# UltronAI/Depth-VO-Feat

Hardware: AMD Instinct MI355X
Metric: KITTI 256x832 stereo-seq samples/sec fwd+bwd (higher is better)
Workload: dtype f32

## Files before the change

### depth-vo-feat_amd/csrc/conv.hip

```cpp
#include "dvf_common.h"
#include "conv_op.h"
#include "conv_pipe_host.h"
#include "conv_gather.h"
#include "conv_wgrad.h"
#include "wgrad_pipe.h"

namespace {

__device__ __forceinline__ float act_grad(float g, float yv, int act, float alpha, float beta) {
    if (act == DVF_ACT_RELU) return (yv > 0.f) ? g : 0.f;
    if (act == DVF_ACT_SIGMOID_AFFINE) {
        const float sg = (yv - beta) / alpha;
        return g * alpha * sg * (1.f - sg);
    }
    return g;
}

template <bool VEC>
__global__ __launch_bounds__(256) void act_bwd_kernel(const float *__restrict__ dy, const float *__restrict__ y,
                                                      float *__restrict__ dpre, float *dbias, int C, int HW, int act,
                                                      float alpha, float beta, int chunks, float *part = nullptr, int nper = 0) {
    __shared__ float red[4];
    const int plane = blockIdx.x / chunks, chunk = blockIdx.x - plane * chunks;
    const int c = plane % C;
// ... 263 lines not shown
    const int rc = plan_gather(op, pl);
    return rc ? rc : pl.ws_floats;
}

struct DgradSeg {
    int s, off;
    ConvOp op;
    bool packed;
    PipePlan plan;
    int64_t packed_off;
};

template <class F>
int for_each_dgrad_seg(const dvf_conv_desc *d, const int *seg_channels, int nseg, bool use_pipe, F visit) {
    DgradSeg v;
    v.off = 0; v.packed_off = 0;
    for (v.s = 0; v.s < nseg; ++v.s) {
        int rc = make_dgrad_op(d, v.off, seg_channels[v.s], v.op);
        v.packed = false;
        if (use_pipe) {
            if (rc) return rc;
            rc = plan_pipe(v.op, v.plan);
            if (rc && rc != DVF_ERR_UNSUPPORTED) return rc;
            v.packed = !rc;
        }
        rc = visit(v);
        if (rc) return rc;
        if (v.packed) v.packed_off += v.plan.packed_floats;
        v.off += seg_channels[v.s];
    }
// ... 13 lines not shown
        if (rc) return rc;
        rc = plan_pipe(op, pl);
        if (rc == DVF_ERR_UNSUPPORTED && want_ws) return unpacked_ws_floats(op, fwd_direct(d, nseg) != FWD_NONE);
        return rc ? rc : (want_ws ? pl.ws_floats : pl.packed_floats);
    }
    if (op_kind != 1) return DVF_ERR_INVALID_ARG;
    int64_t total = 0, wmax = 0;
    int nsup = 0;
    rc = for_each_dgrad_seg(d, seg_channels, nseg, true, [&](const DgradSeg &v) -> int {
        int64_t wf = 0;
        if (v.packed) {
            total += v.plan.packed_floats;
            wf = v.plan.ws_floats;
            ++nsup;
        } else if (want_ws) {
            wf = unpacked_ws_floats(v.op, dvf_head_seg_dgrad_applicable(d, v.op.M));
            if (wf < 0) return (int)wf;
        }
        wmax = wf > wmax ? wf : wmax;
        return DVF_OK;
    });
    if (rc) return rc;
    if (!nsup && !want_ws) return DVF_ERR_UNSUPPORTED;
    return want_ws ? wmax : total;
}

WgradArgs wgrad_args(const dvf_conv_desc *d, const float *const *in_segs, const int *seg_channels, int s, const float *dpre,
                     float *dw) {
    int off = 0;
    for (int i = 0; i < s; ++i) off += seg_channels[i];
    const int segc = s < 0 ? d->C_in : seg_channels[s];
// ... 307 lines not shown
    }
    return fwd_unpacked(d, op, io, seg_channels, nseg, w, ws, ws_floats, st);
}

int dvf_conv2d_dgrad(const dvf_conv_desc *d, const float *dpre, const float *packed, const float *w, float *const *din_segs,
                     const int *seg_channels, int nseg, float *ws, int64_t ws_floats, const float *const *mask_segs,
                     void *stream) {
    dvf_plan_reset();
    int rc = check_desc(d);
    if (rc) return rc;
    rc = check_segs(d, seg_channels, nseg);
    if (rc) return rc;
    if (!dpre || !w || !din_segs) return DVF_ERR_INVALID_ARG;
    hipStream_t st = dvf_stream(stream);
    auto mask = [&](int s) -> const float * { return mask_segs ? mask_segs[s] : nullptr; };
    if (dvf_head_dgrad_applicable(d, nseg) || (dvf_head_applicable(d, nseg) && !packed))
        return din_segs[0] ? dvf_head_dgrad(d, dpre, w, din_segs[0], st, mask(0)) : DVF_OK;
    return for_each_dgrad_seg(d, seg_channels, nseg, packed != nullptr, [&](const DgradSeg &v) -> int {
        if (!din_segs[v.s]) return DVF_OK;
        const ConvIO io{&dpre, nullptr, din_segs[v.s], mask(v.s)};
        int r = v.packed ? run_pipe(v.op, v.plan, io, packed + v.packed_off, ws, ws_floats, st) : DVF_ERR_UNSUPPORTED;
        if (r == DVF_ERR_UNSUPPORTED) r = dgrad_unpacked(d, v.op, io, w, ws, ws_floats, st);
        return r;
    });
}

int dvf_conv2d_pack_jobs(const dvf_conv_desc *d, const int *seg_channels, int nseg, int op_kind, const float *w, float *packed,
                         void *jobs_host, int max_jobs, int *blocks_out, int *lds_bytes_out) {
    static_assert(sizeof(PackArgs) <= DVF_PACK_JOB_BYTES, "DVF_PACK_JOB_BYTES too small");
    int rc = check_desc(d);
    if (rc) return rc;
// ... 54 lines not shown
```

### depth-vo-feat_amd/csrc/conv_head.h

```cpp
#pragma once
#include "dvf_common.h"
bool dvf_head_applicable(const dvf_conv_desc *d, int nseg);
bool dvf_head_fwd_applicable(const dvf_conv_desc *d, int nseg);
bool dvf_head_dgrad_applicable(const dvf_conv_desc *d, int nseg);
int dvf_head_fwd(const dvf_conv_desc *d, const float *in, const float *w, const float *bias, float *out, hipStream_t st);
bool dvf_head_wide_applicable(const dvf_conv_desc *d, int nseg);
int dvf_head_fwd_segs(const dvf_conv_desc *d, const float *const *in_segs, const int *seg_channels, int nseg, const float *w,
                      const float *bias, float *out, hipStream_t st);
int dvf_head_dgrad(const dvf_conv_desc *d, const float *dpre, const float *w, float *din, hipStream_t st, const float *mask = nullptr);
int dvf_head_wgrad(const dvf_conv_desc *d, const float *in, const float *dpre, float *dw, int accumulate, hipStream_t st,
                   float *ws = nullptr, int64_t ws_floats = 0);
int64_t dvf_head_wgrad_ws_floats(const dvf_conv_desc *d);
bool dvf_head_seg_dgrad_applicable(const dvf_conv_desc *d, int segc);
int dvf_head_seg_dgrad(const dvf_conv_desc *d, const float *dpre, const float *w, float *din, int seg_off, int segc,
                       hipStream_t st, const float *mask = nullptr);
bool dvf_dconvt_applicable(const dvf_conv_desc *d, int nseg);
int dvf_dconvt_fwd(const dvf_conv_desc *d, const float *in, const float *w, const float *bias, float *out, hipStream_t st);
```

### depth-vo-feat_amd/csrc/conv_head.hip

```cpp
#include "conv_head.h"
#include "conv_epilogue.h"

namespace {

using dvfp::apply_act;

constexpr int HT_W = 64, HT_H = 4;
constexpr int HP_W = HT_W + 2, HP_H = HT_H + 2;
constexpr int HCK = 8;

__device__ __forceinline__ void stage_tile(float *lds, const float *__restrict__ src, int64_t plane, int nch, int H, int W,
                                           int y0, int x0) {
    for (int e = threadIdx.x; e < nch * HP_H * HP_W; e += 256) {
        const int ch = e / (HP_H * HP_W), r = e - ch * (HP_H * HP_W), py = r / HP_W, px = r - py * HP_W;
        const int y = y0 + py - 1, x = x0 + px - 1;
        lds[e] = (y >= 0 && y < H && x >= 0 && x < W) ? src[ch * plane + (int64_t)y * W + x] : 0.f;
    }
}

template <int ROWS, int MO, class WK>
__device__ __forceinline__ void taps9(const float (&v)[ROWS + 2][3], WK wk, float (&acc)[ROWS][MO]) {
#pragma unroll
    for (int m = 0; m < MO; ++m)
#pragma unroll
        for (int k = 0; k < 9; ++k) {
            const float w = wk(m, k);
#pragma unroll
            for (int r = 0; r < ROWS; ++r) acc[r][m] = fmaf(w, v[k / 3 + r][k % 3], acc[r][m]);
        }
}

constexpr int FT_H = 8;
constexpr int HEAD_MAX_SEGS = 3;
struct HeadSegs {
    const float *p[HEAD_MAX_SEGS];
    int c[HEAD_MAX_SEGS];
    int n;
};
template <int MO, int HCKT, int FTH>
__global__ __launch_bounds__(256) void head_fwd_kernel(const HeadSegs in, const float *__restrict__ w,
                                                       const float *__restrict__ bias, float *__restrict__ out, int C, int H,
                                                       int W, int tilesX, int act, float alpha, float beta, int ws_m, int ws_c,
                                                       int flip, const float *__restrict__ mask) {
    constexpr int ROWS = FTH / 4, FPH = FTH + 2, FPN = FPH * HP_W, FLD = (FPN + 255) / 256;
    extern __shared__ __attribute__((aligned(16))) float wsh[];
    float *tile = wsh + ((MO * C * 9 + 3) & ~3);
    for (int e = threadIdx.x; e < MO * C * 9; e += 256) {
        const int m = e / (C * 9), r = e - m * (C * 9), c = r / 9, k = r - c * 9;
        const float wv = w[(int64_t)m * ws_m + (int64_t)c * ws_c + (flip ? 8 - k : k)];
        if (MO == 16) wsh[(c * MO + m) * 9 + k] = wv;
        else wsh[e] = wv;
    }
    const int n = blockIdx.y, tY = blockIdx.x / tilesX, tX = blockIdx.x - tY * tilesX;
    const int y0 = tY * FTH, x0 = tX * HT_W;
    const int lx = threadIdx.x & (HT_W - 1), ly = (threadIdx.x >> 6) * ROWS;
    const int64_t plane = (int64_t)H * W;
    int soff[FLD];
#pragma unroll
    for (int i = 0; i < FLD; ++i) {
        const int e = threadIdx.x + 256 * i, py = e / HP_W, px = e - py * HP_W;
        const int y = y0 + py - 1, x = x0 + px - 1;
        soff[i] = (e < FPN && y >= 0 && y < H && x >= 0 && x < W) ? y * W + x : -1;
    }
    float acc[ROWS][MO];
#pragma unroll
    for (int m = 0; m < MO; ++m)
// ... 22 lines not shown
        for (int ch = 0; ch < HCKT; ++ch)
#pragma unroll
            for (int i = 0; i < FLD; ++i) {
                const int e = threadIdx.x + 256 * i;
                if (e < FPN) tile[ch * FPN + e] = stg[ch][i];
            }
        __syncthreads();
        if (sg2 < in.n) issue(sg2, cs2);
        auto hood = [&](int ch, float (&v)[ROWS + 2][3]) __attribute__((always_inline)) {
            const float *t = tile + ch * FPN + ly * HP_W + lx;
#pragma unroll
            for (int a = 0; a < ROWS + 2; ++a)
#pragma unroll
                for (int b = 0; b < 3; ++b) v[a][b] = t[a * HP_W + b];
        };
        if constexpr (MO != 16) {
            auto wlds = [&](int c) __attribute__((always_inline)) {
                return [=](int m, int k) __attribute__((always_inline)) { return wsh[(m * C + c) * 9 + k]; };
            };
            float part[3][ROWS][MO];
#pragma unroll
            for (int q = 0; q < 3; ++q)
#pragma unroll
                for (int r = 0; r < ROWS; ++r)
#pragma unroll
                    for (int m = 0; m < MO; ++m) part[q][r][m] = 0.f;
            int ch = 0;
            for (; ch + 4 <= nch; ch += 4) {
                float v4[4][ROWS + 2][3];
#pragma unroll
                for (int q = 0; q < 4; ++q) hood(ch + q, v4[q]);
#pragma unroll
                for (int q = 0; q < 4; ++q)
#pragma unroll
                    for (int m = 0; m < MO; ++m) {
                        const float *wm = wsh + (m * C + cg + ch + q) * 9;
#pragma unroll
                        for (int k = 0; k < 9; ++k) {
                            const float wk = wm[k];
#pragma unroll
                            for (int r = 0; r < ROWS; ++r) {
                                if (q == 0) acc[r][m] = fmaf(wk, v4[q][k / 3 + r][k % 3], acc[r][m]);
                                else part[q - 1][r][m] = fmaf(wk, v4[q][k / 3 + r][k % 3], part[q - 1][r][m]);
                            }
                        }
                    }
            }
            for (; ch < nch; ++ch) {
                float v[ROWS + 2][3];
                hood(ch, v);
                taps9<ROWS, MO>(v, wlds(cg + ch), acc);
            }
#pragma unroll
            for (int r = 0; r < ROWS; ++r)
#pragma unroll
                for (int m = 0; m < MO; ++m) acc[r][m] += (part[0][r][m] + part[1][r][m]) + part[2][r][m];
        } else {
            for (int ch = 0; ch < nch; ++ch) {
                float v[ROWS + 2][3];
                hood(ch, v);
                typedef float f4h __attribute__((ext_vector_type(4)));
                const f4h *wq = reinterpret_cast<const f4h *>(wsh + (cg + ch) * (MO * 9));
                f4h wr[MO * 9 / 4];
#pragma unroll
                for (int q = 0; q < MO * 9 / 4; ++q) wr[q] = wq[q];
                taps9<ROWS, MO>(v, [&](int m, int k) __attribute__((always_inline)) { return wr[(m * 9 + k) >> 2][(m * 9 + k) & 3]; }, acc);
            }
        }
        cg += nch; sg = sg2; cs = cs2;
    }
    const int x = x0 + lx;
#pragma unroll
    for (int r = 0; r < ROWS; ++r) {
        const int y = y0 + ly + r;
        if (y < H && x < W) {
            if (mask) {
#pragma unroll
                for (int m = 0; m < MO; ++m) {
                    const int64_t idx = ((int64_t)n * MO + m) * plane + (int64_t)y * W + x;
                    out[idx] = mask[idx] > 0.f ? acc[r][m] : 0.f;
                }
            } else {
#pragma unroll
                for (int m = 0; m < MO; ++m)
                    out[((int64_t)n * MO + m) * plane + (int64_t)y * W + x] = apply_act(acc[r][m], act, alpha, beta);
            }
        }
    }
}

template <int MO>
__global__ __launch_bounds__(256) void head_dgrad_kernel(const float *__restrict__ dpre, const float *__restrict__ w,
                                                         float *__restrict__ din, int C, int H, int W, int tilesX,
                                                         const float *__restrict__ mask) {
    __shared__ float tile[MO * HP_H * HP_W];
    extern __shared__ __attribute__((aligned(16))) float wsh[];
    constexpr int WPC = (MO * 9 + 3) & ~3;
    for (int e = threadIdx.x; e < C * MO * 9; e += 256) {
        const int c = e / (MO * 9), r = e - c * (MO * 9), m = r / 9, k = r - m * 9;
        wsh[c * WPC + r] = w[((int64_t)m * C + c) * 9 + k];
    }
    const int n = blockIdx.y, tY = blockIdx.x / tilesX, tX = blockIdx.x - tY * tilesX;
    const int y0 = tY * HT_H, x0 = tX * HT_W;
    const int lx = threadIdx.x & (HT_W - 1), ly = threadIdx.x >> 6;
    const int64_t plane = (int64_t)H * W;
    stage_tile(tile, dpre + (int64_t)n * MO * plane, plane, MO, H, W, y0, x0);
    __syncthreads();
    float g[MO][9];
#pragma unroll
    for (int m = 0; m < MO; ++m)
#pragma unroll
        for (int a = 0; a < 3; ++a)
#pragma unroll
            for (int b = 0; b < 3; ++b) g[m][a * 3 + b] = tile[m * (HP_H * HP_W) + (ly + 2 - a) * HP_W + (lx + 2 - b)];
    const int y = y0 + ly, x = x0 + lx;
    if (y >= H || x >= W) return;
    const int64_t base = (int64_t)n * C * plane + (int64_t)y * W + x;
    float *dst = din + base;
    const float *mk = mask ? mask + base : nullptr;
    for (int c0 = 0; c0 < C; c0 += 4) {
        float sv[4], mv[4];
#pragma unroll
        for (int q = 0; q < 4; ++q) {
            const int c = min(c0 + q, C - 1);
            mv[q] = mk ? mk[c * plane] : 1.f;
            const float *wc = wsh + c * WPC;
            float s = 0.f;
#pragma unroll
            for (int m = 0; m < MO; ++m)
#pragma unroll
                for (int k = 0; k < 9; ++k) s = fmaf(wc[m * 9 + k], g[m][k], s);
            sv[q] = s;
        }
#pragma unroll
        for (int q = 0; q < 4; ++q)
            if (c0 + q < C) dst[(c0 + q) * plane] = (mv[q] > 0.f) ? sv[q] : 0.f;
    }
}

template <bool VEC>
__device__ __forceinline__ void hw_load4(const float *__restrict__ p, int x0, int W, bool ok, float (&v)[4]) {
    if (VEC) {
        typedef float f4 __attribute__((ext_vector_type(4)));
        f4 t = {0.f, 0.f, 0.f, 0.f};
        if (ok) t = *reinterpret_cast<const f4 *>(p);
#pragma unroll
        for (int j = 0; j < 4; ++j) v[j] = t[j];
    } else {
#pragma unroll
        for (int j = 0; j < 4; ++j) v[j] = (ok && x0 + j < W) ? p[j] : 0.f;
    }
// ... 95 lines not shown
            const int64_t o = ((int64_t)m * C + c0 + c) * 9 + t;
            if (part) part[(int64_t)blockIdx.y * MO * C * 9 + o] = s;
            else atomicAdd(&dw[o], s);
        }
    }
}

__global__ __launch_bounds__(256) void head_wgrad_finish_kernel(const float *__restrict__ part, float *dw, int n, int groups) {
    const int e = blockIdx.x * 256 + threadIdx.x;
    if (e >= n) return;
    float s = 0.f;
    for (int g = 0; g < groups; ++g) s += part[(int64_t)g * n + e];
    dw[e] += s;
}


template <int CO, int K>
__global__ __launch_bounds__(256) void dconvt_s2_fwd_kernel(const float *__restrict__ in, const float *__restrict__ w,
                                                            const float *__restrict__ bias, float *__restrict__ out, int C, int H,
                                                            int W, int OH, int OW, int act, float alpha, float beta) {
    extern __shared__ __attribute__((aligned(16))) float wlds[];
    constexpr int WPC = CO * K * K;
    static_assert(WPC % 4 == 0, "weights of one input channel are read in 16-byte pieces");
    typedef float f4w __attribute__((ext_vector_type(4)));
    for (int e = threadIdx.x; e < C * WPC / 4; e += 256)
        reinterpret_cast<f4w *>(wlds)[e] = reinterpret_cast<const f4w *>(w)[e];
    __syncthreads();
    const int x = blockIdx.x * 64 + (threadIdx.x & 63), y = blockIdx.y * 4 + (threadIdx.x >> 6), n = blockIdx.z;
    const bool inside = x < W && y < H;
    const bool rok[3] = {y - 1 >= 0 && y - 1 < H, y < H, y + 1 < H}, cok[3] = {x - 1 >= 0 && x - 1 < W, x < W, x + 1 < W};
// ... 51 lines not shown
            } else {
                if (X < OW) q[0] = r0;
                if (X + 1 < OW) q[1] = r1;
            }
        }
    }
}

}

bool dvf_head_applicable(const dvf_conv_desc *d, int nseg) {
    return nseg == 1 && !d->transposed && d->KH == 3 && d->KW == 3 && d->stride == 1 && d->pad == 1 && d->C_out >= 1 &&
           d->C_out <= 4 && d->H_out == d->H_in && d->W_out == d->W_in && d->C_in >= 4 && d->C_in * d->C_out <= 1024 &&
           dvf_tune("DVF_NO_HEAD") == nullptr;
}
bool dvf_head_fwd_applicable(const dvf_conv_desc *d, int nseg) {
    static const int maxc = dvf_tune("DVF_HEAD_FWD_MAXC") ? atoi(dvf_tune("DVF_HEAD_FWD_MAXC")) : 127;
    return dvf_head_applicable(d, nseg) && d->C_in <= maxc;
}
bool dvf_head_dgrad_applicable(const dvf_conv_desc *d, int nseg) {
    static const int maxc = dvf_tune("DVF_HEAD_DGRAD_MAXC") ? atoi(dvf_tune("DVF_HEAD_DGRAD_MAXC")) : 32;
    return dvf_head_applicable(d, nseg) && d->C_in <= maxc;
}

bool dvf_dconvt_applicable(const dvf_conv_desc *d, int nseg) {
    const bool k3 = d->KH == 3 && d->KW == 3, k4 = d->KH == 4 && d->KW == 4;
    return nseg == 1 && d->transposed && d->stride == 2 && d->pad == 1 && (k3 || k4) && d->C_out == 16 &&
           d->C_in >= 8 && d->C_in <= 64 && d->H_out <= 2 * d->H_in && d->W_out <= 2 * d->W_in &&
           (int64_t)d->H_in * d->W_in >= 64 * 64 && (int64_t)d->N * d->C_out * d->H_out * d->W_out < ((int64_t)1 << 31) &&
           dvf_tune("DVF_NO_DCONVT") == nullptr;
}

int dvf_dconvt_fwd(const dvf_conv_desc *d, const float *in, const float *w, const float *bias, float *out, hipStream_t st) {
    const dim3 grid(cdiv(d->W_in, 64), cdiv(d->H_in, 4), d->N);
    const size_t lds = (size_t)d->C_in * d->C_out * d->KH * d->KW * 4;
    if ((reinterpret_cast<uintptr_t>(w) & 15) != 0 || lds > 64 * 1024) return DVF_ERR_UNSUPPORTED;
#define DCONVT(CO, K) dconvt_s2_fwd_kernel<CO, K><<<grid, 256, lds, st>>>(in, w, bias, out, d->C_in, d->H_in, d->W_in, d->H_out, d->W_out, d->act, d->alpha, d->beta)
    if (d->KH == 3) DCONVT(16, 3);
    else DCONVT(16, 4);
#undef DCONVT
    DVF_LAUNCH_CHECK();
    dvf_plan_note(DVF_K_DCONVT_FWD, d->C_out, d->KH);
    return DVF_OK;
}

#define HEAD_CASE(N, ...) case N: { constexpr int MO = N; __VA_ARGS__; } break;
#define HEAD_DISPATCH(MOV, CALL, ...)             \
    switch (MOV) {                               \
        HEAD_CASE(1, CALL) HEAD_CASE(2, CALL) HEAD_CASE(3, CALL) HEAD_CASE(4, CALL) __VA_ARGS__ \
        default: return DVF_ERR_UNSUPPORTED;     \
    }

static int head_fwd_launch(int MOv, const HeadSegs &in, const float *w, const float *bias, float *out, int C, int N, int H, int W,
                           int act, float alpha, float beta, int ws_m, int ws_c, int flip, const float *mask, hipStream_t st) {
    const bool lowres = (int64_t)N * H * W <= (int64_t)4 * 64 * 208 && MOv <= 4 && C >= 32;
    const int FTH = lowres ? 4 : FT_H, HCKT = lowres ? 32 : HCK;
    const int tilesX = cdiv(W, HT_W), tilesY = cdiv(H, FTH);
    const dim3 grid(tilesX * tilesY, N);
    const size_t lds = ((size_t)((MOv * C * 9 + 3) & ~3) + (size_t)HCKT * (FTH + 2) * HP_W) * 4;
#define HEAD_FWD_GO(HC, FH) head_fwd_kernel<MO, HC, FH><<<grid, 256, lds, st>>>(in, w, bias, out, C, H, W, tilesX, act, alpha, beta, ws_m, ws_c, flip, mask)
    if (lowres) {
        static bool big[5] = {false, false, false, false, false};
        HEAD_DISPATCH(MOv, {
            if (lds > 64 * 1024 && !big[MO]) {
                if (hipFuncSetAttribute(reinterpret_cast<const void *>(&head_fwd_kernel<MO, 32, 4>), hipFuncAttributeMaxDynamicSharedMemorySize, 160 * 1024) != hipSuccess) return DVF_ERR_LAUNCH;
                big[MO] = true;
            }
            HEAD_FWD_GO(32, 4); });
    } else {
        HEAD_DISPATCH(MOv, (HEAD_FWD_GO(8, 8)), HEAD_CASE(16, (HEAD_FWD_GO(8, 8))));
    }
#undef HEAD_FWD_GO
    DVF_LAUNCH_CHECK();
    return DVF_OK;
}

int dvf_head_fwd(const dvf_conv_desc *d, const float *in, const float *w, const float *bias, float *out, hipStream_t st) {
    const int one = d->C_in;
    return dvf_head_fwd_segs(d, &in, &one, 1, w, bias, out, st);
}

bool dvf_head_wide_applicable(const dvf_conv_desc *d, int nseg) {
    return nseg >= 1 && nseg <= HEAD_MAX_SEGS && !d->transposed && d->KH == 3 && d->KW == 3 && d->stride == 1 && d->pad == 1 &&
           d->C_out == 16 && d->C_in <= 24 && d->H_out == d->H_in && d->W_out == d->W_in &&
           (int64_t)d->H_in * d->W_in >= 64 * 64 && dvf_tune("DVF_NO_HEAD") == nullptr && dvf_tune("DVF_NO_WIDE_HEAD") == nullptr;
}

// ... 19 lines not shown

int dvf_head_seg_dgrad(const dvf_conv_desc *d, const float *dpre, const float *w, float *din, int seg_off, int segc,
                       hipStream_t st, const float *mask) {
    const float *wseg = w + (int64_t)seg_off * 9;
    HeadSegs in{};
    for (int s = 0; s < HEAD_MAX_SEGS; ++s) { in.p[s] = dpre; in.c[s] = s == 0 ? d->C_out : 0; }
    in.n = 1;
    const int rc = head_fwd_launch(segc, in, wseg, nullptr, din, d->C_out, d->N, d->H_in, d->W_in, DVF_ACT_NONE, 1.f, 0.f, 9,
                                   d->C_in * 9, 1, mask, st);
    if (rc) return rc;
    dvf_plan_note(DVF_K_HEAD_SEG_DGRAD, segc);
    return DVF_OK;
}

int dvf_head_dgrad(const dvf_conv_desc *d, const float *dpre, const float *w, float *din, hipStream_t st, const float *mask) {
    const int tilesX = cdiv(d->W_in, HT_W), tilesY = cdiv(d->H_in, HT_H);
    const dim3 grid(tilesX * tilesY, d->N);
    HEAD_DISPATCH(d->C_out, (head_dgrad_kernel<MO><<<grid, 256, (size_t)d->C_in * ((MO * 9 + 3) & ~3) * 4, st>>>(
                                dpre, w, din, d->C_in, d->H_in, d->W_in, tilesX, mask)));
    DVF_LAUNCH_CHECK();
    dvf_plan_note(DVF_K_HEAD_DGRAD, d->C_out);
    return DVF_OK;
}

struct HeadWgradGrid { int cch, RS, xgroups, segs, chunks, groups; int64_t units; };
static HeadWgradGrid head_wgrad_grid(const dvf_conv_desc *d) {
    HeadWgradGrid g;
    g.xgroups = cdiv(d->W_in, 4);
    auto blocks = [&](int cch, int rs) {
        return (int64_t)cdiv(d->C_in, cch) * (((int64_t)d->N * cdiv(d->H_in, rs) * g.xgroups + 255) / 256);
    };
    const int min_blocks = 400, max_blocks = 1024;
    g.cch = (d->C_out <= 2 && blocks(4, 8) >= 512) ? 4 : 2;
    g.RS = 8;
// ... 41 lines not shown
```

### depth-vo-feat_amd/csrc/conv_op.h

```cpp
#pragma once
#include "dvf_common.h"
#include "conv_head.h"

namespace {

inline int ilog2(int v) { int l = 0; while ((1 << l) < v) ++l; return l; }
inline int roundup(int v, int q) { return (v + q - 1) / q * q; }

struct ClassSpec { int OS, py, px, IS, by, bx, TA, TB, OHc, OWc; int tapmap[49]; };

struct ConvOp {
    int nseg, segC[DVF_MAX_SEGS];
    int w_mode;
    int Mtot, Rtot, KK, m_base, M;
    int N, IH, IW, OH, OW;
    int act;
    float alpha, beta;
    ClassSpec cls[4];
    int ncls;
    bool covers;
    int Tmax, TAmax, TBmax, OHc, OWc;
    bool head_fwd;
};

struct ConvIO {
    const float *const *in;
    const float *bias;
    float *out;
    const float *mask;
};

int check_desc(const dvf_conv_desc *d) {
    if (!d) return DVF_ERR_INVALID_ARG;
    if (d->N <= 0 || d->C_in <= 0 || d->C_out <= 0 || d->H_in <= 0 || d->W_in <= 0 || d->H_out <= 0 || d->W_out <= 0)
        return DVF_ERR_INVALID_ARG;
    if (d->KH < 1 || d->KW < 1 || d->KH > 7 || d->KW > 7 || (d->stride != 1 && d->stride != 2) || d->pad < 0)
        return DVF_ERR_INVALID_ARG;
// ... 55 lines not shown
    for (int i = 0; i < op.ncls; ++i) {
        const ClassSpec &c = op.cls[i];
        op.Tmax = max(op.Tmax, c.TA * c.TB); op.TAmax = max(op.TAmax, c.TA); op.TBmax = max(op.TBmax, c.TB);
        op.OHc = max(op.OHc, c.OHc); op.OWc = max(op.OWc, c.OWc);
    }
    return op.ncls >= 1 ? DVF_OK : DVF_ERR_UNSUPPORTED;
}

int make_fwd_op(const dvf_conv_desc *d, const int *seg_channels, int nseg, ConvOp &op) {
    op = ConvOp{};
    for (int s = 0; s < nseg; ++s) op.segC[s] = seg_channels[s];
    op.nseg = nseg; op.M = d->C_out;
    op.N = d->N; op.IH = d->H_in; op.IW = d->W_in; op.OH = d->H_out; op.OW = d->W_out;
    op.act = d->act; op.alpha = d->alpha; op.beta = d->beta;
    op.KK = d->KH * d->KW; op.m_base = 0; op.Mtot = d->C_out; op.Rtot = d->C_in;
    op.head_fwd = !dvf_head_fwd_applicable(d, nseg) && dvf_head_applicable(d, nseg);
    op.w_mode = d->transposed ? 1 : 0;
    return set_classes(d, !d->transposed, op);
}

int make_dgrad_op(const dvf_conv_desc *d, int off, int segc, ConvOp &op) {
    op = ConvOp{};
    op.segC[0] = d->C_out; op.nseg = 1; op.M = segc;
    op.N = d->N; op.IH = d->H_out; op.IW = d->W_out; op.OH = d->H_in; op.OW = d->W_in;
    op.act = DVF_ACT_NONE;
    op.KK = d->KH * d->KW; op.m_base = off; op.Mtot = d->C_in; op.Rtot = d->C_out;
    op.head_fwd = false;
    op.w_mode = d->transposed ? 0 : 1;
    return set_classes(d, d->transposed != 0, op);
}

}
```

### depth-vo-feat_amd/csrc/conv_pipe_host.h

```cpp
#pragma once
#include <string.h>
#include "dvf_common.h"
#include "conv_pipe.h"
#include "conv_op.h"

namespace {

using dvfp::PClass;
using dvfp::PipeArgs;
using dvfp::PipeGeo;
using dvfp::pipe_geo;
using dvfp::PIPE_MAXNPI;
using dvfp::OUT_FUSED;
using dvfp::OUT_ATOMIC;
using dvfp::OUT_WS;

struct alignas(8) PackArgsBody {
    const float *w;
    float *wp;
    int w_mode;
    int Mtot, Rtot, KK, m_base, M;
    int nseg, segC[DVF_MAX_SEGS];
    int ncls, NCH, CK, MB, VW, TBU;
    int TB[4], TA[4];
// ... 271 lines not shown
                    const double cov = (double)cdiv(OWc, BW) * BW * cdiv(OHc, BH) * BH * cdiv(N, BN) * BN;
                    const double narrow = (SW >= 16 ? 0.0 : (SW == 8 ? 0.12 : 0.3)) + (BW >= 32 ? 0.0 : 0.08);
                    const double cost = cov * (1.0 + narrow + 0.02 * lsh + 0.02 * lsn) + 1e-3 * (BW + BH);
                    if (cost < best.cov) best = PipeTiles{lsw, lsh, TGX, TGY, TGN, BN, cost};
                }
            }
        }
    }
    return best;
}


int plan_pipe(const ConvOp &op, PipePlan &pl) {
    if (op.ncls < 1) return DVF_ERR_UNSUPPORTED;
    const ClassSpec *cls = op.cls;
    const int ncls = op.ncls, Tmax = op.Tmax, TAmax = op.TAmax, TBmax = op.TBmax, OHc = op.OHc, OWc = op.OWc;
    const bool head_fwd = op.head_fwd;
    PipeArgs &a = pl.a;
    a = PipeArgs{};
    for (int s = 0; s < op.nseg; ++s) a.segC[s] = op.segC[s];
    a.nseg = op.nseg; a.M = op.M;
    a.N = op.N; a.IH = op.IH; a.IW = op.IW; a.OH = op.OH; a.OW = op.OW;
    a.act = op.act; a.alpha = op.alpha; a.beta = op.beta;
    a.ncls = ncls; a.OS = cls[0].OS; a.IS = cls[0].IS;
    const PipeOverride ov = pipe_override();
    static const int smallm = dvf_tune("DVF_PIPE_SMALLM") ? atoi(dvf_tune("DVF_PIPE_SMALLM")) : 0;
    int ctot = 0;
    for (int s = 0; s < a.nseg; ++s) ctot += a.segC[s];
    static const int headc = dvf_tune("DVF_PIPE_HEADC") ? atoi(dvf_tune("DVF_PIPE_HEADC")) : 128;
    const bool wide_head = head_fwd && a.M <= 4 && ncls == 1 && ctot >= headc && Tmax == 9;
    const bool small_ok = a.M > 16 || wide_head || (!(smallm & 8) && a.M <= 16 && ncls > 1) ||
                          ((smallm & 2) && a.M <= 16) || ((smallm & 4) && a.M > 16);
    if (a.M <= 32 && !ov.on && !small_ok) return DVF_ERR_UNSUPPORTED;
    if (ov.on && ov.KS < 0) return DVF_ERR_UNSUPPORTED;
    int maxc = 0;
    for (int s = 0; s < a.nseg; ++s) maxc = a.segC[s] > maxc ? a.segC[s] : maxc;
    const int64_t px = (int64_t)OHc * OWc;
    int TBU = TBmax;
    if (TBU == 6) TBU = 7;
    if (TBU > 7) return DVF_ERR_UNSUPPORTED;
    int MT = a.M > 32 ? 2 : 1;
    int BN = 1;
    if (px <= 64) { while (BN < a.N && BN * px < 128 && BN < 32) BN *= 2; }
    int WM = 1;
    if (px * BN <= 64 && a.M >= 128) WM = 2;
    int NT = 2;
// ... 195 lines not shown
```

Measured before the change: 646.3.

## Replace LDS-tiled head conv kernels with register-streaming fwd/dgrad kernels

Adds new streaming kernels for the 1-4 output-channel head convolutions, covering both forward and dgrad. Each lane computes a 4-wide by RS-row output strip held in registers, with double-buffered channel loads and weights broadcast via readlane. Forward can split channels across waves with an LDS reduction, and dgrad splits channels across grid.y, so small spatial sizes still fill the GPU. Every head layer, including wide ones, now routes to these kernels instead of the packed pipe GEMM or the LDS-tile kernels. This risks slower paths for large-C layers that previously used the pipe, and adds more register pressure.

New measurement: 651.0, median of 6. No clear change (+0.7%).

```diff
diff --git a/depth-vo-feat_amd/csrc/conv.hip b/depth-vo-feat_amd/csrc/conv.hip
--- a/depth-vo-feat_amd/csrc/conv.hip
+++ b/depth-vo-feat_amd/csrc/conv.hip
@@ -301,6 +301,7 @@
 template <class F>
 int for_each_dgrad_seg(const dvf_conv_desc *d, const int *seg_channels, int nseg, bool use_pipe, F visit) {
     DgradSeg v;
+    use_pipe = use_pipe && !dvf_head_applicable(d, nseg);
     v.off = 0; v.packed_off = 0;
     for (v.s = 0; v.s < nseg; ++v.s) {
         int rc = make_dgrad_op(d, v.off, seg_channels[v.s], v.op);
@@ -344,7 +345,7 @@
             wf = v.plan.ws_floats;
             ++nsup;
         } else if (want_ws) {
-            wf = unpacked_ws_floats(v.op, dvf_head_seg_dgrad_applicable(d, v.op.M));
+            wf = unpacked_ws_floats(v.op, dvf_head_applicable(d, nseg) || dvf_head_seg_dgrad_applicable(d, v.op.M));
             if (wf < 0) return (int)wf;
         }
         wmax = wf > wmax ? wf : wmax;
@@ -682,7 +683,7 @@
     if (!dpre || !w || !din_segs) return DVF_ERR_INVALID_ARG;
     hipStream_t st = dvf_stream(stream);
     auto mask = [&](int s) -> const float * { return mask_segs ? mask_segs[s] : nullptr; };
-    if (dvf_head_dgrad_applicable(d, nseg) || (dvf_head_applicable(d, nseg) && !packed))
+    if (dvf_head_applicable(d, nseg))
         return din_segs[0] ? dvf_head_dgrad(d, dpre, w, din_segs[0], st, mask(0)) : DVF_OK;
     return for_each_dgrad_seg(d, seg_channels, nseg, packed != nullptr, [&](const DgradSeg &v) -> int {
         if (!din_segs[v.s]) return DVF_OK;
diff --git a/depth-vo-feat_amd/csrc/conv_head.h b/depth-vo-feat_amd/csrc/conv_head.h
--- a/depth-vo-feat_amd/csrc/conv_head.h
+++ b/depth-vo-feat_amd/csrc/conv_head.h
@@ -1,8 +1,6 @@
 #pragma once
 #include "dvf_common.h"
 bool dvf_head_applicable(const dvf_conv_desc *d, int nseg);
-bool dvf_head_fwd_applicable(const dvf_conv_desc *d, int nseg);
-bool dvf_head_dgrad_applicable(const dvf_conv_desc *d, int nseg);
 int dvf_head_fwd(const dvf_conv_desc *d, const float *in, const float *w, const float *bias, float *out, hipStream_t st);
 bool dvf_head_wide_applicable(const dvf_conv_desc *d, int nseg);
 int dvf_head_fwd_segs(const dvf_conv_desc *d, const float *const *in_segs, const int *seg_channels, int nseg, const float *w,
diff --git a/depth-vo-feat_amd/csrc/conv_head.hip b/depth-vo-feat_amd/csrc/conv_head.hip
--- a/depth-vo-feat_amd/csrc/conv_head.hip
+++ b/depth-vo-feat_amd/csrc/conv_head.hip
@@ -5,18 +5,9 @@
 
 using dvfp::apply_act;
 
-constexpr int HT_W = 64, HT_H = 4;
-constexpr int HP_W = HT_W + 2, HP_H = HT_H + 2;
+constexpr int HT_W = 64;
+constexpr int HP_W = HT_W + 2;
 constexpr int HCK = 8;
-
-__device__ __forceinline__ void stage_tile(float *lds, const float *__restrict__ src, int64_t plane, int nch, int H, int W,
-                                           int y0, int x0) {
-    for (int e = threadIdx.x; e < nch * HP_H * HP_W; e += 256) {
-        const int ch = e / (HP_H * HP_W), r = e - ch * (HP_H * HP_W), py = r / HP_W, px = r - py * HP_W;
-        const int y = y0 + py - 1, x = x0 + px - 1;
-        lds[e] = (y >= 0 && y < H && x >= 0 && x < W) ? src[ch * plane + (int64_t)y * W + x] : 0.f;
-    }
-}
 
 template <int ROWS, int MO, class WK>
 __device__ __forceinline__ void taps9(const float (&v)[ROWS + 2][3], WK wk, float (&acc)[ROWS][MO]) {
@@ -45,11 +36,10 @@
     constexpr int ROWS = FTH / 4, FPH = FTH + 2, FPN = FPH * HP_W, FLD = (FPN + 255) / 256;
     extern __shared__ __attribute__((aligned(16))) float wsh[];
     float *tile = wsh + ((MO * C * 9 + 3) & ~3);
+    static_assert(MO == 16, "the 1-4 channel layers run head_stream_fwd_kernel");
     for (int e = threadIdx.x; e < MO * C * 9; e += 256) {
         const int m = e / (C * 9), r = e - m * (C * 9), c = r / 9, k = r - c * 9;
-        const float wv = w[(int64_t)m * ws_m + (int64_t)c * ws_c + (flip ? 8 - k : k)];
-        if (MO == 16) wsh[(c * MO + m) * 9 + k] = wv;
-        else wsh[e] = wv;
+        wsh[(c * MO + m) * 9 + k] = w[(int64_t)m * ws_m + (int64_t)c * ws_c + (flip ? 8 - k : k)];
     }
     const int n = blockIdx.y, tY = blockIdx.x / tilesX, tX = blockIdx.x - tY * tilesX;
     const int y0 = tY * FTH, x0 = tX * HT_W;
@@ -102,58 +92,15 @@
 #pragma unroll
                 for (int b = 0; b < 3; ++b) v[a][b] = t[a * HP_W + b];
         };
-        if constexpr (MO != 16) {
-            auto wlds = [&](int c) __attribute__((always_inline)) {
-                return [=](int m, int k) __attribute__((always_inline)) { return wsh[(m * C + c) * 9 + k]; };
-            };
-            float part[3][ROWS][MO];
-#pragma unroll
-            for (int q = 0; q < 3; ++q)
-#pragma unroll
-                for (int r = 0; r < ROWS; ++r)
-#pragma unroll
-                    for (int m = 0; m < MO; ++m) part[q][r][m] = 0.f;
-            int ch = 0;
-            for (; ch + 4 <= nch; ch += 4) {
-                float v4[4][ROWS + 2][3];
-#pragma unroll
-                for (int q = 0; q < 4; ++q) hood(ch + q, v4[q]);
-#pragma unroll
-                for (int q = 0; q < 4; ++q)
-#pragma unroll
-                    for (int m = 0; m < MO; ++m) {
-                        const float *wm = wsh + (m * C + cg + ch + q) * 9;
-#pragma unroll
-                        for (int k = 0; k < 9; ++k) {
-                            const float wk = wm[k];
-#pragma unroll
-                            for (int r = 0; r < ROWS; ++r) {
-                                if (q == 0) acc[r][m] = fmaf(wk, v4[q][k / 3 + r][k % 3], acc[r][m]);
-                                else part[q - 1][r][m] = fmaf(wk, v4[q][k / 3 + r][k % 3], part[q - 1][r][m]);
-                            }
-                        }
-                    }
-            }
-            for (; ch < nch; ++ch) {
-                float v[ROWS + 2][3];
-                hood(ch, v);
-                taps9<ROWS, MO>(v, wlds(cg + ch), acc);
-            }
-#pragma unroll
-            for (int r = 0; r < ROWS; ++r)
-#pragma unroll
-                for (int m = 0; m < MO; ++m) acc[r][m] += (part[0][r][m] + part[1][r][m]) + part[2][r][m];
-        } else {
-            for (int ch = 0; ch < nch; ++ch) {
-                float v[ROWS + 2][3];
-                hood(ch, v);
-                typedef float f4h __attribute__((ext_vector_type(4)));
-                const f4h *wq = reinterpret_cast<const f4h *>(wsh + (cg + ch) * (MO * 9));
-                f4h wr[MO * 9 / 4];
-#pragma unroll
-                for (int q = 0; q < MO * 9 / 4; ++q) wr[q] = wq[q];
-                taps9<ROWS, MO>(v, [&](int m, int k) __attribute__((always_inline)) { return wr[(m * 9 + k) >> 2][(m * 9 + k) & 3]; }, acc);
-            }
+        for (int ch = 0; ch < nch; ++ch) {
+            float v[ROWS + 2][3];
+            hood(ch, v);
+            typedef float f4h __attribute__((ext_vector_type(4)));
+            const f4h *wq = reinterpret_cast<const f4h *>(wsh + (cg + ch) * (MO * 9));
+            f4h wr[MO * 9 / 4];
+#pragma unroll
+            for (int q = 0; q < MO * 9 / 4; ++q) wr[q] = wq[q];
+            taps9<ROWS, MO>(v, [&](int m, int k) __attribute__((always_inline)) { return wr[(m * 9 + k) >> 2][(m * 9 + k) & 3]; }, acc);
         }
         cg += nch; sg = sg2; cs = cs2;
     }
@@ -174,55 +121,6 @@
                     out[((int64_t)n * MO + m) * plane + (int64_t)y * W + x] = apply_act(acc[r][m], act, alpha, beta);
             }
         }
-    }
-}
-
-template <int MO>
-__global__ __launch_bounds__(256) void head_dgrad_kernel(const float *__restrict__ dpre, const float *__restrict__ w,
-                                                         float *__restrict__ din, int C, int H, int W, int tilesX,
-                                                         const float *__restrict__ mask) {
-    __shared__ float tile[MO * HP_H * HP_W];
-    extern __shared__ __attribute__((aligned(16))) float wsh[];
-    constexpr int WPC = (MO * 9 + 3) & ~3;
-    for (int e = threadIdx.x; e < C * MO * 9; e += 256) {
-        const int c = e / (MO * 9), r = e - c * (MO * 9), m = r / 9, k = r - m * 9;
-        wsh[c * WPC + r] = w[((int64_t)m * C + c) * 9 + k];
-    }
-    const int n = blockIdx.y, tY = blockIdx.x / tilesX, tX = blockIdx.x - tY * tilesX;
-    const int y0 = tY * HT_H, x0 = tX * HT_W;
-    const int lx = threadIdx.x & (HT_W - 1), ly = threadIdx.x >> 6;
-    const int64_t plane = (int64_t)H * W;
-    stage_tile(tile, dpre + (int64_t)n * MO * plane, plane, MO, H, W, y0, x0);
-    __syncthreads();
-    float g[MO][9];
-#pragma unroll
-    for (int m = 0; m < MO; ++m)
-#pragma unroll
-        for (int a = 0; a < 3; ++a)
-#pragma unroll
-            for (int b = 0; b < 3; ++b) g[m][a * 3 + b] = tile[m * (HP_H * HP_W) + (ly + 2 - a) * HP_W + (lx + 2 - b)];
-    const int y = y0 + ly, x = x0 + lx;
-    if (y >= H || x >= W) return;
-    const int64_t base = (int64_t)n * C * plane + (int64_t)y * W + x;
-    float *dst = din + base;
-    const float *mk = mask ? mask + base : nullptr;
-    for (int c0 = 0; c0 < C; c0 += 4) {
-        float sv[4], mv[4];
-#pragma unroll
-        for (int q = 0; q < 4; ++q) {
-            const int c = min(c0 + q, C - 1);
-            mv[q] = mk ? mk[c * plane] : 1.f;
-            const float *wc = wsh + c * WPC;
-            float s = 0.f;
-#pragma unroll
-            for (int m = 0; m < MO; ++m)
-#pragma unroll
-                for (int k = 0; k < 9; ++k) s = fmaf(wc[m * 9 + k], g[m][k], s);
-            sv[q] = s;
-        }
-#pragma unroll
-        for (int q = 0; q < 4; ++q)
-            if (c0 + q < C) dst[(c0 + q) * plane] = (mv[q] > 0.f) ? sv[q] : 0.f;
     }
 }
 
@@ -348,6 +246,251 @@
     dw[e] += s;
 }
 
+
+__device__ __forceinline__ int64_t hs_block() { return (int64_t)(blockIdx.x & 7) * (gridDim.x >> 3) + (blockIdx.x >> 3); }
+
+constexpr int hs_cb(int MO, int RS) { return RS >= 4 ? (MO <= 2 ? 2 : 1) : RS == 2 ? 2 : 4; }
+
+template <bool VEC>
+__device__ __forceinline__ void hs_row6(const float *__restrict__ p, const float *__restrict__ safe, int x0, int W, bool ok,
+                                        float (&x)[6]) {
+    const bool l = ok && x0 > 0, r = ok && x0 + 4 < W;
+    const float vl = *(l ? p - 1 : safe), vr = *(r ? p + 4 : safe);
+    if (VEC) {
+        typedef float f4 __attribute__((ext_vector_type(4)));
+        const f4 t = *reinterpret_cast<const f4 *>(ok ? p : safe);
+#pragma unroll
+        for (int j = 0; j < 4; ++j) x[1 + j] = ok ? t[j] : 0.f;
+    } else {
+#pragma unroll
+        for (int j = 0; j < 4; ++j) {
+            const bool okj = ok && x0 + j < W;
+            const float t = *(okj ? p + j : safe);
+            x[1 + j] = okj ? t : 0.f;
+        }
+    }
+    x[0] = l ? vl : 0.f;
+    x[5] = r ? vr : 0.f;
+}
+
+template <int MO, int RS, bool VEC>
+__global__ __launch_bounds__(256) void head_stream_fwd_kernel(const float *__restrict__ in, const float *__restrict__ w,
+                                                              const float *__restrict__ bias, float *__restrict__ out, int C,
+                                                              int H, int W, int xgroups, int segs, int64_t units, int KS, int act,
+                                                              float alpha, float beta, int ws_m, int ws_c, int flip,
+                                                              const float *__restrict__ mask) {
+    constexpr int CB = hs_cb(MO, RS), NR = RS + 2, NA = RS * 4 * MO;
+    typedef float f4 __attribute__((ext_vector_type(4)));
+    extern __shared__ __attribute__((aligned(16))) float red[];
+    const int wave = __builtin_amdgcn_readfirstlane(threadIdx.x >> 6), lane = threadIdx.x & 63;
+    const int ks = wave & (KS - 1), ug = wave / KS;
+    if (hs_block() * (256 / KS) >= units) return;
+    const int64_t u = (hs_block() * (4 / KS) + ug) * 64 + lane;
+    const bool live = u < units;
+    const int upi = segs * xgroups;
+    const int n = live ? (int)(u / upi) : 0, q = live ? (int)(u - (int64_t)n * upi) : 0;
+    const int seg = q / xgroups, xg = q - seg * xgroups;
+    const int y0 = seg * RS, x0 = xg * 4;
+    const int64_t plane = (int64_t)H * W;
+    const int cper = (C + KS - 1) / KS, cb = ks * cper, ce = min(C, cb + cper);
+    const int64_t ibase = (int64_t)n * C * plane + x0;
+    bool yok[NR];
+#pragma unroll
+    for (int i = 0; i < NR; ++i) yok[i] = live && y0 - 1 + i >= 0 && y0 - 1 + i < H;
+    auto load = [&](int c0, float (&x)[CB][NR][6]) __attribute__((always_inline)) {
+#pragma unroll
+        for (int b = 0; b < CB; ++b) {
+            const bool okc = c0 + b < ce;
+#pragma unroll
+            for (int i = 0; i < NR; ++i)
+                hs_row6<VEC>(in + ibase + (int64_t)(c0 + b) * plane + (int64_t)(y0 - 1 + i) * W, in, x0, W, okc && yok[i], x[b][i]);
+        }
+    };
+    const int wl = min(lane, MO * 9 - 1), wm = wl / 9;
+    const int64_t woff = (int64_t)wm * ws_m + (flip ? 8 - (wl - wm * 9) : wl - wm * 9);
+    auto load_w = [&](int c0, float (&wv)[CB]) __attribute__((always_inline)) {
+#pragma unroll
+        for (int b = 0; b < CB; ++b) wv[b] = w[(int64_t)min(c0 + b, ce - 1) * ws_c + woff];
+    };
+    float acc[RS][4][MO];
+#pragma unroll
+    for (int m = 0; m < MO; ++m) {
+        const float b0 = (bias && ks == 0) ? bias[m] : 0.f;
+#pragma unroll
+        for (int r = 0; r < RS; ++r)
+#pragma unroll
+            for (int j = 0; j < 4; ++j) acc[r][j][m] = b0;
+    }
+    auto fma = [&](int c0, const float (&x)[CB][NR][6], const float (&wv)[CB]) __attribute__((always_inline)) {
+#pragma unroll
+        for (int b = 0; b < CB; ++b) {
+            if (c0 + b >= ce) continue;
+            float wk[MO][9];
+#pragma unroll
+            for (int m = 0; m < MO; ++m)
+#pragma unroll
+                for (int k = 0; k < 9; ++k) wk[m][k] = __int_as_float(__builtin_amdgcn_readlane(__float_as_int(wv[b]), m * 9 + k));
+#pragma unroll
+            for (int m = 0; m < MO; ++m)
+#pragma unroll
+                for (int ta = 0; ta < 3; ++ta)
+#pragma unroll
+                    for (int tb = 0; tb < 3; ++tb)
+#pragma unroll
+                        for (int r = 0; r < RS; ++r)
+#pragma unroll
+                            for (int j = 0; j < 4; ++j)
+                                acc[r][j][m] = fmaf(wk[m][ta * 3 + tb], x[b][r + ta][j + tb], acc[r][j][m]);
+        }
+    };
+    float xa[CB][NR][6], xb[CB][NR][6], wa[CB], wb[CB];
+    load_w(cb, wa);
+    load(cb, xa);
+    for (int c0 = cb; c0 < ce; c0 += 2 * CB) {
+        load_w(c0 + CB, wb);
+        load(c0 + CB, xb);
+        fma(c0, xa, wa);
+        load_w(c0 + 2 * CB, wa);
+        load(c0 + 2 * CB, xa);
+        fma(c0 + CB, xb, wb);
+    }
+    if (KS > 1) {
+        if (ks > 0) {
+            float *r = red + (int64_t)(ug * (KS - 1) + ks - 1) * NA * 64 + lane;
+#pragma unroll
+            for (int a = 0; a < NA; ++a) r[a * 64] = acc[a / (4 * MO)][(a / MO) & 3][a % MO];
+        }
+        __syncthreads();
+        if (ks > 0) return;
+        for (int k = 1; k < KS; ++k) {
+            const float *r = red + (int64_t)(ug * (KS - 1) + k - 1) * NA * 64 + lane;
+#pragma unroll
+            for (int a = 0; a < NA; ++a) acc[a / (4 * MO)][(a / MO) & 3][a % MO] += r[a * 64];
+        }
+    }
+    if (!live) return;
+#pragma unroll
+    for (int r = 0; r < RS; ++r) {
+        const int y = y0 + r;
+        if (y >= H) continue;
+#pragma unroll
+        for (int m = 0; m < MO; ++m) {
+            const int64_t idx = ((int64_t)n * MO + m) * plane + (int64_t)y * W + x0;
+            float o[4];
+            if (mask) {
+                float mv[4];
+                hw_load4<VEC>(mask + idx, x0, W, true, mv);
+#pragma unroll
+                for (int j = 0; j < 4; ++j) o[j] = mv[j] > 0.f ? acc[r][j][m] : 0.f;
+            } else {
+#pragma unroll
+                for (int j = 0; j < 4; ++j) o[j] = apply_act(acc[r][j][m], act, alpha, beta);
+            }
+            if (VEC) {
+                f4 t = {o[0], o[1], o[2], o[3]};
+                *reinterpret_cast<f4 *>(out + idx) = t;
+            } else {
+#pragma unroll
+                for (int j = 0; j < 4; ++j)
+                    if (x0 + j < W) out[idx + j] = o[j];
+            }
+        }
+    }
+}
+
+template <int MO, bool VEC>
+__global__ __launch_bounds__(256) void head_stream_dgrad_kernel(const float *__restrict__ dpre, const float *__restrict__ w,
+                                                                float *__restrict__ din, int C, int H, int W, int xgroups,
+                                                                int64_t units, int cper, const float *__restrict__ mask) {
+    constexpr int CQ = 4;
+    typedef float f4 __attribute__((ext_vector_type(4)));
+    if (hs_block() * 256 >= units) return;
+    const int64_t u = hs_block() * 256 + threadIdx.x;
+    const bool live = u < units;
+    const int upi = H * xgroups;
+    const int n = live ? (int)(u / upi) : 0, q = live ? (int)(u - (int64_t)n * upi) : 0;
+    const int y = q / xgroups, xg = q - y * xgroups, x0 = xg * 4;
+    const int64_t plane = (int64_t)H * W;
+    float g[MO][3][6];
+#pragma unroll
+    for (int m = 0; m < MO; ++m)
+#pragma unroll
+        for (int a = 0; a < 3; ++a) {
+            const int r = y - 1 + a;
+            hs_row6<VEC>(dpre + ((int64_t)n * MO + m) * plane + (int64_t)r * W + x0, dpre, x0, W, live && r >= 0 && r < H, g[m][a]);
+        }
+    const int cb = blockIdx.y * cper, ce = min(C, cb + cper);
+    const int64_t base = (int64_t)n * C * plane + (int64_t)y * W + x0;
+    auto load_mask = [&](int c0, float (&mv)[CQ][4]) __attribute__((always_inline)) {
+#pragma unroll
+        for (int b = 0; b < CQ; ++b) {
+            const bool ok = mask && live && c0 + b < ce;
+            const float *p = mask + base + (int64_t)(c0 + b) * plane;
+            if (VEC) {
+                const f4 t = *reinterpret_cast<const f4 *>(ok ? p : dpre);
+#pragma unroll
+                for (int j = 0; j < 4; ++j) mv[b][j] = ok ? t[j] : 1.f;
+            } else {
+#pragma unroll
+                for (int j = 0; j < 4; ++j) {
+                    const bool okj = ok && x0 + j < W;
+                    const float t = *(okj ? p + j : dpre);
+                    mv[b][j] = okj ? t : 1.f;
+                }
+            }
+        }
+    };
+    const int lane = threadIdx.x & 63, wl = min(lane, MO * 9 - 1), wm = wl / 9;
+    const int64_t woff = (int64_t)wm * C * 9 + (wl - wm * 9);
+    auto load_w = [&](int c0, float (&wv)[CQ]) __attribute__((always_inline)) {
+#pragma unroll
+        for (int b = 0; b < CQ; ++b) wv[b] = w[(int64_t)min(c0 + b, ce - 1) * 9 + woff];
+    };
+    float mv[CQ][4], mn[CQ][4], wv[CQ], wn[CQ];
+    load_mask(cb, mv);
+    load_w(cb, wv);
+    for (int c0 = cb; c0 < ce; c0 += CQ) {
+        load_mask(c0 + CQ, mn);
+        load_w(c0 + CQ, wn);
+#pragma unroll
+        for (int b = 0; b < CQ; ++b) {
+            const int c = c0 + b;
+            if (c >= ce) continue;
+            float wk[MO][9];
+#pragma unroll
+            for (int m = 0; m < MO; ++m)
+#pragma unroll
+                for (int k = 0; k < 9; ++k) wk[m][k] = __int_as_float(__builtin_amdgcn_readlane(__float_as_int(wv[b]), m * 9 + k));
+            float s[4] = {0.f, 0.f, 0.f, 0.f};
+#pragma unroll
+            for (int m = 0; m < MO; ++m)
+#pragma unroll
+                for (int ta = 0; ta < 3; ++ta)
+#pragma unroll
+                    for (int tb = 0; tb < 3; ++tb)
+#pragma unroll
+                        for (int j = 0; j < 4; ++j) s[j] = fmaf(wk[m][ta * 3 + tb], g[m][2 - ta][j + 2 - tb], s[j]);
+#pragma unroll
+            for (int j = 0; j < 4; ++j) s[j] = mv[b][j] > 0.f ? s[j] : 0.f;
+            float *dst = din + base + (int64_t)c * plane;
+            if (!live) continue;
+            if (VEC) {
+                f4 t = {s[0], s[1], s[2], s[3]};
+                *reinterpret_cast<f4 *>(dst) = t;
+            } else {
+#pragma unroll
+                for (int j = 0; j < 4; ++j)
+                    if (x0 + j < W) dst[j] = s[j];
+            }
+        }
+#pragma unroll
+        for (int b = 0; b < CQ; ++b)
+#pragma unroll
+            for (int j = 0; j < 4; ++j) mv[b][j] = mn[b][j];
+#pragma unroll
+        for (int b = 0; b < CQ; ++b) wv[b] = wn[b];
+    }
+}
 
 template <int CO, int K>
 __global__ __launch_bounds__(256) void dconvt_s2_fwd_kernel(const float *__restrict__ in, const float *__restrict__ w,
@@ -429,15 +572,6 @@
            d->C_out <= 4 && d->H_out == d->H_in && d->W_out == d->W_in && d->C_in >= 4 && d->C_in * d->C_out <= 1024 &&
            dvf_tune("DVF_NO_HEAD") == nullptr;
 }
-bool dvf_head_fwd_applicable(const dvf_conv_desc *d, int nseg) {
-    static const int maxc = dvf_tune("DVF_HEAD_FWD_MAXC") ? atoi(dvf_tune("DVF_HEAD_FWD_MAXC")) : 127;
-    return dvf_head_applicable(d, nseg) && d->C_in <= maxc;
-}
-bool dvf_head_dgrad_applicable(const dvf_conv_desc *d, int nseg) {
-    static const int maxc = dvf_tune("DVF_HEAD_DGRAD_MAXC") ? atoi(dvf_tune("DVF_HEAD_DGRAD_MAXC")) : 32;
-    return dvf_head_applicable(d, nseg) && d->C_in <= maxc;
-}
-
 bool dvf_dconvt_applicable(const dvf_conv_desc *d, int nseg) {
     const bool k3 = d->KH == 3 && d->KW == 3, k4 = d->KH == 4 && d->KW == 4;
     return nseg == 1 && d->transposed && d->stride == 2 && d->pad == 1 && (k3 || k4) && d->C_out == 16 &&
@@ -466,26 +600,49 @@
         default: return DVF_ERR_UNSUPPORTED;     \
     }
 
+struct HeadStreamGrid { int RS, KS, xgroups, segs; int64_t units, blocks; };
+static HeadStreamGrid head_stream_grid(int C, int N, int H, int W) {
+    HeadStreamGrid g;
+    g.xgroups = cdiv(W, 4);
+    auto blocks = [&](int rs, int ks) { return ((int64_t)N * cdiv(H, rs) * g.xgroups + 256 / ks - 1) / (256 / ks); };
+    const int min_blocks = 400;
+    g.RS = 4; g.KS = 1;
+    while (blocks(g.RS, g.KS) < min_blocks) {
+        if (g.KS < 4 && C >= 8 * g.KS) g.KS *= 2;
+        else if (g.RS > 1) g.RS >>= 1;
+        else break;
+    }
+    if (const char *t = dvf_tune("DVF_HEAD_FS_RS")) g.RS = atoi(t) == 1 || atoi(t) == 2 ? atoi(t) : 4;
+    if (const char *t = dvf_tune("DVF_HEAD_FS_KS")) g.KS = atoi(t) == 2 || atoi(t) == 4 ? atoi(t) : 1;
+    g.segs = cdiv(H, g.RS);
+    g.units = (int64_t)N * g.segs * g.xgroups;
+    g.blocks = blocks(g.RS, g.KS);
+    return g;
+}
+
 static int head_fwd_launch(int MOv, const HeadSegs &in, const float *w, const float *bias, float *out, int C, int N, int H, int W,
                            int act, float alpha, float beta, int ws_m, int ws_c, int flip, const float *mask, hipStream_t st) {
-    const bool lowres = (int64_t)N * H * W <= (int64_t)4 * 64 * 208 && MOv <= 4 && C >= 32;
-    const int FTH = lowres ? 4 : FT_H, HCKT = lowres ? 32 : HCK;
-    const int tilesX = cdiv(W, HT_W), tilesY = cdiv(H, FTH);
-    const dim3 grid(tilesX * tilesY, N);
-    const size_t lds = ((size_t)((MOv * C * 9 + 3) & ~3) + (size_t)HCKT * (FTH + 2) * HP_W) * 4;
-#define HEAD_FWD_GO(HC, FH) head_fwd_kernel<MO, HC, FH><<<grid, 256, lds, st>>>(in, w, bias, out, C, H, W, tilesX, act, alpha, beta, ws_m, ws_c, flip, mask)
-    if (lowres) {
-        static bool big[5] = {false, false, false, false, false};
-        HEAD_DISPATCH(MOv, {
-            if (lds > 64 * 1024 && !big[MO]) {
-                if (hipFuncSetAttribute(reinterpret_cast<const void *>(&head_fwd_kernel<MO, 32, 4>), hipFuncAttributeMaxDynamicSharedMemorySize, 160 * 1024) != hipSuccess) return DVF_ERR_LAUNCH;
-                big[MO] = true;
-            }
-            HEAD_FWD_GO(32, 4); });
-    } else {
-        HEAD_DISPATCH(MOv, (HEAD_FWD_GO(8, 8)), HEAD_CASE(16, (HEAD_FWD_GO(8, 8))));
-    }
-#undef HEAD_FWD_GO
+    if (MOv == 16) {
+        const int tilesX = cdiv(W, HT_W), tilesY = cdiv(H, FT_H);
+        const dim3 grid(tilesX * tilesY, N);
+        const size_t lds = ((size_t)((MOv * C * 9 + 3) & ~3) + (size_t)HCK * (FT_H + 2) * HP_W) * 4;
+        head_fwd_kernel<16, HCK, FT_H><<<grid, 256, lds, st>>>(in, w, bias, out, C, H, W, tilesX, act, alpha, beta, ws_m, ws_c, flip, mask);
+        DVF_LAUNCH_CHECK();
+        return DVF_OK;
+    }
+    if (in.n != 1) return DVF_ERR_UNSUPPORTED;
+    const HeadStreamGrid g = head_stream_grid(C, N, H, W);
+    if (g.blocks > 0x7ffffff0) return DVF_ERR_UNSUPPORTED;
+    const unsigned nblk = (unsigned)((g.blocks + 7) & ~(int64_t)7);
+    const bool vec = W % 4 == 0 && ((reinterpret_cast<uintptr_t>(in.p[0]) | reinterpret_cast<uintptr_t>(out) |
+                                     reinterpret_cast<uintptr_t>(mask)) & 15) == 0;
+    const size_t lds = (size_t)(4 - 4 / g.KS) * g.RS * 4 * MOv * 256;
+#define HEAD_FS_GO(RS, VEC) head_stream_fwd_kernel<MO, RS, VEC><<<nblk, 256, lds, st>>>(in.p[0], w, bias, out, C, H, W, g.xgroups, g.segs, g.units, g.KS, act, alpha, beta, ws_m, ws_c, flip, mask)
+    HEAD_DISPATCH(MOv, {
+        if (g.RS == 4) { if (vec) HEAD_FS_GO(4, true); else HEAD_FS_GO(4, false); }
+        else if (g.RS == 2) { if (vec) HEAD_FS_GO(2, true); else HEAD_FS_GO(2, false); }
+        else { if (vec) HEAD_FS_GO(1, true); else HEAD_FS_GO(1, false); } });
+#undef HEAD_FS_GO
     DVF_LAUNCH_CHECK();
     return DVF_OK;
 }
@@ -535,10 +692,18 @@
 }
 
 int dvf_head_dgrad(const dvf_conv_desc *d, const float *dpre, const float *w, float *din, hipStream_t st, const float *mask) {
-    const int tilesX = cdiv(d->W_in, HT_W), tilesY = cdiv(d->H_in, HT_H);
-    const dim3 grid(tilesX * tilesY, d->N);
-    HEAD_DISPATCH(d->C_out, (head_dgrad_kernel<MO><<<grid, 256, (size_t)d->C_in * ((MO * 9 + 3) & ~3) * 4, st>>>(
-                                dpre, w, din, d->C_in, d->H_in, d->W_in, tilesX, mask)));
+    const int xgroups = cdiv(d->W_in, 4);
+    const int64_t units = (int64_t)d->N * d->H_in * xgroups, bx = (units + 255) / 256;
+    if (bx > 0x7ffffff0) return DVF_ERR_UNSUPPORTED;
+    int split = 1;
+    while (bx * split < 400 && cdiv(d->C_in, split * 2) >= 4) split *= 2;
+    const int cper = (cdiv(d->C_in, split) + 3) & ~3;
+    const dim3 grid((unsigned)((bx + 7) & ~(int64_t)7), cdiv(d->C_in, cper));
+    const bool vec = d->W_in % 4 == 0 && ((reinterpret_cast<uintptr_t>(dpre) | reinterpret_cast<uintptr_t>(din) |
+                                           reinterpret_cast<uintptr_t>(mask)) & 15) == 0;
+#define HEAD_DG_GO(VEC) head_stream_dgrad_kernel<MO, VEC><<<grid, 256, 0, st>>>(dpre, w, din, d->C_in, d->H_in, d->W_in, xgroups, units, cper, mask)
+    HEAD_DISPATCH(d->C_out, { if (vec) HEAD_DG_GO(true); else HEAD_DG_GO(false); });
+#undef HEAD_DG_GO
     DVF_LAUNCH_CHECK();
     dvf_plan_note(DVF_K_HEAD_DGRAD, d->C_out);
     return DVF_OK;
diff --git a/depth-vo-feat_amd/csrc/conv_op.h b/depth-vo-feat_amd/csrc/conv_op.h
--- a/depth-vo-feat_amd/csrc/conv_op.h
+++ b/depth-vo-feat_amd/csrc/conv_op.h
@@ -20,7 +20,6 @@
     int ncls;
     bool covers;
     int Tmax, TAmax, TBmax, OHc, OWc;
-    bool head_fwd;
 };
 
 struct ConvIO {
@@ -106,7 +105,6 @@
     op.N = d->N; op.IH = d->H_in; op.IW = d->W_in; op.OH = d->H_out; op.OW = d->W_out;
     op.act = d->act; op.alpha = d->alpha; op.beta = d->beta;
     op.KK = d->KH * d->KW; op.m_base = 0; op.Mtot = d->C_out; op.Rtot = d->C_in;
-    op.head_fwd = !dvf_head_fwd_applicable(d, nseg) && dvf_head_applicable(d, nseg);
     op.w_mode = d->transposed ? 1 : 0;
     return set_classes(d, !d->transposed, op);
 }
@@ -117,7 +115,6 @@
     op.N = d->N; op.IH = d->H_out; op.IW = d->W_out; op.OH = d->H_in; op.OW = d->W_in;
     op.act = DVF_ACT_NONE;
     op.KK = d->KH * d->KW; op.m_base = off; op.Mtot = d->C_in; op.Rtot = d->C_out;
-    op.head_fwd = false;
     op.w_mode = d->transposed ? 0 : 1;
     return set_classes(d, d->transposed != 0, op);
 }
diff --git a/depth-vo-feat_amd/csrc/conv_pipe_host.h b/depth-vo-feat_amd/csrc/conv_pipe_host.h
--- a/depth-vo-feat_amd/csrc/conv_pipe_host.h
+++ b/depth-vo-feat_amd/csrc/conv_pipe_host.h
@@ -309,8 +309,7 @@
 int plan_pipe(const ConvOp &op, PipePlan &pl) {
     if (op.ncls < 1) return DVF_ERR_UNSUPPORTED;
     const ClassSpec *cls = op.cls;
-    const int ncls = op.ncls, Tmax = op.Tmax, TAmax = op.TAmax, TBmax = op.TBmax, OHc = op.OHc, OWc = op.OWc;
-    const bool head_fwd = op.head_fwd;
+    const int ncls = op.ncls, TAmax = op.TAmax, TBmax = op.TBmax, OHc = op.OHc, OWc = op.OWc;
     PipeArgs &a = pl.a;
     a = PipeArgs{};
     for (int s = 0; s < op.nseg; ++s) a.segC[s] = op.segC[s];
@@ -320,11 +319,7 @@
     a.ncls = ncls; a.OS = cls[0].OS; a.IS = cls[0].IS;
     const PipeOverride ov = pipe_override();
     static const int smallm = dvf_tune("DVF_PIPE_SMALLM") ? atoi(dvf_tune("DVF_PIPE_SMALLM")) : 0;
-    int ctot = 0;
-    for (int s = 0; s < a.nseg; ++s) ctot += a.segC[s];
-    static const int headc = dvf_tune("DVF_PIPE_HEADC") ? atoi(dvf_tune("DVF_PIPE_HEADC")) : 128;
-    const bool wide_head = head_fwd && a.M <= 4 && ncls == 1 && ctot >= headc && Tmax == 9;
-    const bool small_ok = a.M > 16 || wide_head || (!(smallm & 8) && a.M <= 16 && ncls > 1) ||
+    const bool small_ok = a.M > 16 || (!(smallm & 8) && a.M <= 16 && ncls > 1) ||
                           ((smallm & 2) && a.M <= 16) || ((smallm & 4) && a.M > 16);
     if (a.M <= 32 && !ov.on && !small_ok) return DVF_ERR_UNSUPPORTED;
     if (ov.on && ov.KS < 0) return DVF_ERR_UNSUPPORTED;
```
